# netsniff-ng/netsniff-ng

Hardware: AMD Instinct MI355X
Metric: Mpkt/s + GB/s device-resident dissect, 64B & IMIX; bit-exact fields vs ref (higher is better)
Workload: dtype u8

## Files before the change

### netsniff-ng_amd/csrc/nsd_fast.h

```cpp
#ifndef NSD_FAST_H
#define NSD_FAST_H

#include "nsd_fused.h"

namespace nsd {


constexpr int FROW = WIN1 / 4;

struct FastShared {
	alignas(16) uint32_t win[WAVES][64 * FROW];
	unsigned long long cnt[NSD_NCOUNTERS];
	uint32_t ops[32];
	uint8_t lay3[256];
	uint32_t pcnt[WAVES];
};

__device__ __forceinline__ void stage_write_sw(uint32_t *wwin, const Chunks<WIN1> &ch, int lane)
{
#pragma unroll
	for (int r = 0; r < 4; r++) {
		const int t = r * 64 + lane;
		const int q = t / 4, c = t % 4;
		const uint32_t nv = (ch.nv >> (8 * r)) & 0xFF;
		uint32_t w[4] = { ch.v[r].x, ch.v[r].y, ch.v[r].z, ch.v[r].w };
		if (nv < 16) {
#pragma unroll
			for (int j = 0; j < 4; j++) {
				const uint32_t bp = 4 * j;
				if (bp >= nv)
					w[j] = 0;
				else if (bp + 4 > nv)
					w[j] &= (1u << ((nv - bp) * 8)) - 1u;
			}
		}
		*(uint4 *)(wwin + q * FROW + ((c ^ swz_of((uint32_t)q, 4)) << 2)) = make_uint4(w[0], w[1], w[2], w[3]);
	}
}

__device__ __forceinline__ uint32_t fold_weighted(uint32_t sum, bool odd)
{
	sum = (sum >> 16) + (sum & 0xFFFF);
	sum = (sum >> 16) + (sum & 0xFFFF);
	return odd ? ((sum & 0xFF) << 8 | sum >> 8) : sum;
}

static_assert(k_plain_lay3[6] == NSD_OPS_TCP && k_plain_lay3[17] == NSD_OPS_UDP,
	      "plain_walk's protocol map differs from eth_lay3");

__device__ __forceinline__ bool plain_is(const LSrc<true, WIN1> &s, uint32_t caplen)
{
	const uint32_t r = s.m + 12, j = r >> 2, sh = r & 3;
	const uint32_t d12 = __builtin_amdgcn_alignbyte(s.dw(j + 1), s.dw(j), sh);
	const uint32_t d20 = __builtin_amdgcn_alignbyte(s.dw(j + 3), s.dw(j + 2), sh);
	const uint32_t proto = d20 >> 24;
	return caplen >= 42 && (d12 & 0xFFFFFFu) == 0x450008u && (proto == 6 || proto == 17);
}

__device__ __forceinline__ void plain_walk(const LSrc<true, WIN1> &s, uint32_t caplen, WalkOut &w)
{
	const uint32_t r = s.m + 12, j = r >> 2, sh = r & 3;
	const uint32_t w0 = s.dw(j), w1 = s.dw(j + 1), w2 = s.dw(j + 2), w3 = s.dw(j + 3), w4 = s.dw(j + 4),
		       w5 = s.dw(j + 5), w6 = s.dw(j + 6);
	const uint32_t d12 = __builtin_amdgcn_alignbyte(w1, w0, sh), d16 = __builtin_amdgcn_alignbyte(w2, w1, sh),
		       d20 = __builtin_amdgcn_alignbyte(w3, w2, sh), d24 = __builtin_amdgcn_alignbyte(w4, w3, sh),
		       d28 = __builtin_amdgcn_alignbyte(w5, w4, sh), d32 = __builtin_amdgcn_alignbyte(w6, w5, sh);
	uint32_t sum = (d12 >> 16) + (d32 & 0xFFFF);
	sum = __builtin_amdgcn_sad_u16(d16, 0u, sum);
	sum = __builtin_amdgcn_sad_u16(d20, 0u, sum);
	sum = __builtin_amdgcn_sad_u16(d24, 0u, sum);
	sum = __builtin_amdgcn_sad_u16(d28, 0u, sum);
	sum = (sum >> 16) + (sum & 0xffff);
	sum += sum >> 16;
	w.ip_csum = (uint16_t)~sum;
	const int32_t x = (int32_t)__builtin_bswap16((uint16_t)d16) - 20;
	if (x >= 0 && (uint32_t)x < caplen - 34)
		w.tail = 34 + (uint32_t)x;
	const bool tcp = (d20 >> 24) == 6;
	const int l4 = tcp ? NSD_OPS_TCP : NSD_OPS_UDP;
	w.chain = NSD_OPS_ETHERNET | NSD_OPS_IPV4 << 5 | (uint32_t)l4 << 10;
	w.offA = (uint64_t)14 << 16 | (uint64_t)34 << 32;
	w.n = 3;
	const uint32_t len = w.tail - 34, hl = tcp ? 20u : 8u;
	w.data = len >= hl ? 34 + hl : 34;
}

template <int MODE, bool CR>
__device__ __forceinline__ void fast_tiles(FastShared &sh, const uint8_t *__restrict__ frames,
					   const uint64_t *__restrict__ desc, uint32_t n, int start_id,
					   void *__restrict__ rec, const uint32_t *__restrict__ sll, uint32_t *__restrict__ side,
					   uint4 *__restrict__ list, uint32_t cap, uint32_t &ndef, uint32_t &nicmp,
					   uint32_t *__restrict__ heads, uint32_t tail0, uint32_t nheads)
{
	const int lane = threadIdx.x & 63;
	const int wv = __builtin_amdgcn_readfirstlane((int)(threadIdx.x >> 6));
	const uint32_t stride = gridDim.x * BLOCK;
	FlagCnt fc;
	auto uni = [](uint32_t x) -> uint32_t { return (uint32_t)__builtin_amdgcn_readfirstlane((int)x); };
	uint32_t base = uni(blockIdx.x * BLOCK + wv * 64);

	if (MODE != PRINT_NORM && MODE != PRINT_LESS) {
		for (; base < n; base += stride) {
			const uint32_t i = base + lane;
			fc.pkts += FlagCnt::pc(i < n);
			if (i < n) {
				const uint32_t caplen = NSD_DESC_CAPLEN(desc[i]);
				if constexpr (CR)
					__builtin_nontemporal_store(v2u{ 0u, 0u }, (v2u *)rec + i);
				else
					store_rec((uint4 *)rec, i, make_uint4(0, caplen << 16, 0, 0));
				fc.bytes += caplen;
			}
		}
		fc.flush(sh.cnt, lane);
		return;
	}
	if (base >= n)
		return;
	uint32_t *const rows = &sh.win[wv][0];
	auto dsc = [&](uint32_t b) -> uint64_t {
		return desc[b < n && b + lane < n ? b + lane : n - 1];
	};
	auto tile = [&](Chunks<WIN1> &ch, const uint64_t d0, const uint64_t dpre) {
		const uint32_t i = base + lane;
		const bool valid = i < n;
		const uint64_t off = NSD_DESC_OFF(d0);
		const uint32_t caplen = NSD_DESC_CAPLEN(d0);
		WalkOut w;
		walk_init(w, caplen, valid ? start_id : 0);
		stage_write_sw(rows, ch, lane);
		stage_load<WIN1, true>(ch, frames, dpre, lane);
		wave_sync_lds();
		uint32_t fw = FW_DONE;
		const LSrc<true, WIN1> src{ rows + lane * FROW, sh.lay3, nullptr, frames + off, caplen,
					    (uint32_t)off & 15, 0, false, swz_of((uint32_t)lane, 4) << 2 };
		const bool plain = MODE == PRINT_NORM && start_id == NSD_OPS_ETHERNET &&
				   __ballot(valid && !plain_is(src, caplen)) == 0;
		if (plain) {
			if (valid)
				plain_walk(src, caplen, w);
		} else if (valid) {
			fw = fast_walk<MODE, true>(src, caplen, w);
		}
		const bool deferred = fw != FW_DONE;
		wave_sync_lds();
		const bool done = valid && !deferred;
		if (plain) {
			const uint64_t vm = __ballot(valid), tm = __ballot(valid && w.chain >> 10 == NSD_OPS_TCP);
			const uint32_t nv = (uint32_t)__popcll(vm), nt = (uint32_t)__popcll(tm);
			if (lane == 0) {
				atomicAdd(&sh.ops[NSD_OPS_ETHERNET], nv);
				atomicAdd(&sh.ops[NSD_OPS_IPV4], nv);
				if (nt)
					atomicAdd(&sh.ops[NSD_OPS_TCP], nt);
				if (nv - nt)
					atomicAdd(&sh.ops[NSD_OPS_UDP], nv - nt);
			}
			if (valid)
				put_rec_st<CR>(rec, i, w);
			fc.pkts += nv;
			fc.ipbad += FlagCnt::pc(valid && w.ip_csum != 0);
			fc.trim += FlagCnt::pc(valid && w.tail < caplen);
			if (valid)
				fc.bytes += caplen;
			return;
		}
		if (MODE == PRINT_NORM) {
			const bool pnd = w.icmp_pend && done;
			const uint64_t pm = __ballot(pnd);
			if (pnd) {
				const uint32_t part = fold_weighted(w.icmp_sum, ((uint32_t)off + w.icmp_off) & 1);
				uint4 *e = list + (size_t)(cap - 1 - (nicmp + lanes_below(pm))) * SW;
				st_b128(e, make_uint4(i, w.icmp_off | w.icmp_len << 16, part, 0));
				st_b128(e + 1, make_uint4((uint32_t)d0, (uint32_t)(d0 >> 32), 0, 0));
			}
			nicmp = uni(nicmp + (uint32_t)__popcll(pm));
		}
		{
			uint32_t key = done ? w.chain : 0xFFFFFFFFu;
			for (int it = 0;; it++) {
				const uint64_t pm = __ballot(key != 0xFFFFFFFFu);
				if (!pm)
					break;
				if (it == 2) {
					if (key != 0xFFFFFFFFu)
						for (uint32_t k = 0; k < w.n; k++)
							atomicAdd(&sh.ops[(key >> (5 * k)) & 31], 1u);
					break;
				}
				const int leader = __ffsll((unsigned long long)pm) - 1;
				const uint32_t lk = __shfl(key, leader, 64);
				const uint64_t m = __ballot(key == lk);
				if (lane == leader) {
					const uint32_t cnt = (uint32_t)__popcll(m);
					for (uint32_t k = 0, nl = w.n; k < nl; k++)
						atomicAdd(&sh.ops[(lk >> (5 * k)) & 31], cnt);
				}
				if (key == lk)
					key = 0xFFFFFFFFu;
			}
		}
		if (CR && side && done && (w.flags & NSD_F_HOST)) {
			st_b32(side + i, w.data);
			w.flags |= NSD_F_LEAF_END;
		}
		if (done)
			put_rec_st<CR>(rec, i, w);
		fc.add(w, caplen, done);
		const uint64_t dm = __ballot(deferred);
		if (dm) {
			if (deferred) {
				if (fw == FW_RESTART) {
					walk_init(w, caplen, start_id);
					if (start_id == NSD_OPS_SLL) {
						const uint32_t w0 = sll ? sll[5 * (size_t)i] : 0u;
						const uint32_t w2 = sll ? sll[5 * (size_t)i + 2] : 0u;
						const uint32_t proto = __builtin_bswap16((uint16_t)(w0 >> 16));
						w.chain = NSD_OPS_SLL;
						w.n = 1;
						atomicAdd(&sh.ops[NSD_OPS_SLL], 1u);
						w.id = sll_next(w2 & 0xFFFF, proto, MODE, c_lay2h.e[NSD_L2H(proto)]);
					}
				} else {
					for (uint32_t k = 0; k < w.n; k++)
						atomicAdd(&sh.ops[(w.chain >> (5 * k)) & 31], 1u);
				}
				uint4 *e = list + (size_t)(ndef + lanes_below(dm)) * SW;
				st_b128(e, make_uint4(i, w.data | w.tail << 16,
						      (uint32_t)w.ip_csum | (uint32_t)w.flags << 16 | w.n << 24 |
							      (uint32_t)w.id << 27,
						      w.chain));
				const uint32_t offs = CR ? 0u
							 : ((uint32_t)(w.offA >> 16) & 0xFF) | ((uint32_t)(w.offA >> 32) & 0xFF) << 8 |
								   ((uint32_t)(w.offA >> 48) & 0xFF) << 16 | (w.offB & 0xFF) << 24;
				st_b128(e + 1, make_uint4((uint32_t)d0, (uint32_t)(d0 >> 32), offs, 0));
			}
			ndef = uni(ndef + (uint32_t)__popcll(dm));
		}
	};
	const uint32_t ntiles = (n + 63) / 64;
	const uint32_t slim = heads ? tail0 * 64 : n;
	uint32_t cur = heads ? blockIdx.x % nheads : 0, tries = nheads > 1 ? 0 : NSD_TAIL_TRIES;
	bool more = heads != nullptr, asked = false;
	uint32_t gv = 0;
	auto draw = [&]() {
		if (lane == 0) {
			uint32_t z;
			asm volatile("v_mov_b32 %0, 0" : "=v"(z));
			gv = atomicAdd(heads + LINE_WORDS * cur + z, 1u);
		}
	};
	auto ask = [&]() {
		asked = more && ndef + nicmp + 64u * 7 <= cap;
		more = asked;
		if (asked)
			draw();
	};
	uint32_t second = n;
	auto take = [&]() -> uint32_t {
		if (!asked)
			return n;
		asked = false;
		auto tile_of = [&]() -> uint32_t {
			const uint32_t k = (uint32_t)__builtin_amdgcn_readfirstlane((int)gv);
			return tail0 + 2 * (cur + k * nheads);
		};
		uint32_t t = tile_of();
		auto next = [&]() {
			tries++;
			cur = cur + 1 == nheads ? 0 : cur + 1;
			draw();
			t = tile_of();
		};
		static_assert(NSD_TAIL_TRIES == 3, "take(): one nested test per try");
		if (t >= ntiles && tries < NSD_TAIL_TRIES) {
			next();
			if (t >= ntiles && tries < NSD_TAIL_TRIES) {
				next();
				if (t >= ntiles && tries < NSD_TAIL_TRIES)
					next();
			}
		}
		if (t >= ntiles) {
			more = false;
			return n;
		}
		second = t + 1 < ntiles ? (t + 1) * 64 : n;
		if (second == n)
			more = false;
		return t * 64;
	};
	uint32_t nxt = uni(base + 3 * stride);
	auto step = [&]() -> uint32_t {
		uint32_t b;
		if (nxt < slim) {
			b = nxt;
			nxt = uni(nxt + stride);
			if (nxt >= slim)
				ask();
		} else if (second < n) {
			b = second;
			second = n;
		} else {
			b = take();
			ask();
		}
		return b;
	};
	uint32_t b1 = base + stride < slim ? base + stride : n, b2 = base + 2 * stride < slim ? base + 2 * stride : n;
	uint64_t d0 = dsc(base), d1 = dsc(b1), d2 = dsc(b2);
	Chunks<WIN1> chA, chB;
	stage_load<WIN1, true>(chA, frames, d0, lane);
	stage_load<WIN1, true>(chB, frames, d1, lane);
	for (;;) {
		uint32_t b3 = uni(step());
		uint64_t d3 = dsc(b3);
		tile(chA, d0, d2);
		d0 = d1;
		d1 = d2;
		d2 = d3;
		base = uni(b1);
		b1 = b2;
		b2 = b3;
		if (base >= n)
			break;
		b3 = uni(step());
		d3 = dsc(b3);
		tile(chB, d0, d2);
		d0 = d1;
		d1 = d2;
		d2 = d3;
		base = uni(b1);
		b1 = b2;
		b2 = b3;
		if (base >= n)
			break;
	}
	drain_stores();
	if (lane == 0 && ndef + nicmp > cap)
		atomicAdd(&sh.cnt[NSD_CNT_LISTOVF], 1ull);
	fc.flush(sh.cnt, lane);
}

template <int U, bool CR>
__device__ __forceinline__ void fast_icmp_pass(FastShared &sh, const uint8_t *__restrict__ frames,
					       const uint64_t *__restrict__ desc, void *__restrict__ rec,
					       const uint4 *__restrict__ lists, uint32_t cap)
{
	const int lane = threadIdx.x & 63;
	const int wv = threadIdx.x >> 6;
	const uint32_t sub = lane & 3, grp = lane >> 2;
	uint32_t bad = 0;
	for (int l = 0; l < WAVES; l++) {
		const uint32_t cnt = sh.pcnt[l];
		const uint4 *list = lists + ((size_t)blockIdx.x * WAVES + l) * cap * SW;
		for (uint32_t k0 = 64 * ((wv + l) % WAVES); k0 < cnt; k0 += 64 * WAVES) {
			const bool on = k0 + lane < cnt;
			const uint4 *ep = list + (size_t)(cap - 1 - (k0 + lane)) * SW;
			const uint4 e = on ? ep[0] : make_uint4(0, 0, 0, 0);
			const uint32_t i = e.x;
			const uint64_t a = (on ? NSD_DESC_OFF((uint64_t)ep[1].y << 32 | ep[1].x) : 0) + (e.y & 0xFFFF);
			const uint32_t nb = e.y >> 16;
			for (uint32_t q = 0; q < 64 && k0 + q < cnt; q += 16) {
				const int src = (int)(q + grp);
				const uint32_t alo = __shfl((uint32_t)a, src, 64);
				const uint32_t ahi = __shfl((uint32_t)(a >> 32), src, 64);
				const uint32_t mnb = __shfl(nb, src, 64);
				const uint32_t part = __shfl(e.z, src, 64);
				const bool mon = k0 + (uint32_t)src < cnt;
				const uint32_t s0 = alo & 15, endb = s0 + mnb;
				const uint32_t nch = mon ? (endb + 15) >> 4 : 0u;
				const uint4 *base = (const uint4 *)(frames + ((((uint64_t)ahi << 32) | alo) & ~15ull));
				uint32_t sum = sub == 0 ? part : 0u;
				const uint32_t je = sub == 0 ? 0u : nch - 1;
				if ((sub == 0 && nch > 0) || (sub == 1 && nch > 1))
					sum += csum_chunk(base[je], 16 * je, s0, endb);
				for (uint32_t j = 1 + sub; __ballot(j + 1 < nch); j += 4 * U) {
					uint4 v[U];
#pragma unroll
					for (int u = 0; u < U; u++) {
						const uint32_t jj = j + 4 * u;
						v[u] = jj + 1 < nch ? base[jj] : make_uint4(0, 0, 0, 0);
					}
#pragma unroll
					for (int u = 0; u < U; u++) {
						sum = sum_halves(v[u].x, sum);
						sum = sum_halves(v[u].y, sum);
						sum = sum_halves(v[u].z, sum);
						sum = sum_halves(v[u].w, sum);
					}
				}
				sum = (sum >> 16) + (sum & 0xffff);
				sum += __shfl_xor(sum, 1, 64);
				sum += __shfl_xor(sum, 2, 64);
				const uint32_t mi = __shfl(i, src, 64);
				const bool isbad = mon && sub == 0 && csum_final(sum) != 0;
				if (isbad) {
					uint8_t *nf = (uint8_t *)rec + nflags_at<CR>(mi);
					*nf = *nf | NSD_F_ICMP_BAD;
				}
				bad += FlagCnt::pc(isbad);
			}
		}
	}
	if (lane == 0 && bad)
		atomicAdd(&sh.cnt[NSD_CNT_ICMP_BAD], (unsigned long long)bad);
}

template <int MODE, bool CR>
__device__ __forceinline__ void walk_lists(Shared &sh, uint32_t *s_touch, const uint8_t *__restrict__ frames,
					   const uint64_t *__restrict__ desc, uint32_t n, void *__restrict__ rec,
					   uint32_t *__restrict__ ext, uint32_t ext_words, uint32_t *__restrict__ ext_used,
					   uint32_t chunk, unsigned long long *__restrict__ counters,
					   const uint4 *__restrict__ list, uint32_t cnt, uint64_t *__restrict__ pend,
					   uint32_t region)
{
	if (threadIdx.x < 64)
		sh.step[threadIdx.x] = threadIdx.x < 32 ? c_step[threadIdx.x] : c_lay2h.e[threadIdx.x - 32];
	if (threadIdx.x < 32)
		sh.ops[threadIdx.x] = 0;
	if (threadIdx.x < 2 * WAVES)
		sh.wc[threadIdx.x >> 1][threadIdx.x & 1] = 0;
	block_init(sh.cnt, sh.lay3);
	const int lane = threadIdx.x & 63, wv = threadIdx.x >> 6;
	const uint32_t gw = blockIdx.x * WAVES + wv;
	Pending pq{ pend + (size_t)gw * (region / WAVES), region / WAVES, 0, 0 };
	const bool side = CR && ext_words >= n;
	const GenSink<CR> g{ ext, ext_words, ext_used, chunk, &sh.wc[wv][0], sh.ops, &sh.lay[wv][0],
			     CR ? n : 0u, side ? ext : nullptr };
	FlagCnt fc;
	Walker wk;
	walk_init(wk.w, 0, 0);
	wk.d = 0;
	wk.i = 0;
	wk.wb = 0;
	wk.wl = 0;
	wk.have = false;
	wk.stage = false;
	WalkOut pw;
	walk_init(pw, 0, 0);
	RingSt rs;
	rs.init();

	auto load = [&](uint32_t k0, uint4 &x0, uint4 &x1) {
		x0 = x1 = make_uint4(0, 0, 0, 0);
		if (k0 + lane < cnt) {
			const uint4 *e = list + (size_t)(k0 + lane) * SW;
			x0 = e[0];
			x1 = e[1];
		}
	};
	uint4 c0, c1, n0, n1;
	load(0, c0, c1);
	load(64, n0, n1);
	for (uint32_t k0 = 0; k0 < cnt; k0 += 64) {
		{
			const uint64_t d = (uint64_t)n1.y << 32 | n1.x;
			const uint32_t m = (uint32_t)NSD_DESC_OFF(d) & 15, caplen = NSD_DESC_CAPLEN(d);
			const uint32_t wb = ((n0.y & 0xFFFF) + m) & ~15u;
			const bool on = k0 + 64 + lane < cnt && wb < caplen + m;
			const uint64_t a = (uint64_t)frames + (NSD_DESC_OFF(d) & ~15ull) + wb;
			const bool two = on && (a & 127) != 0 && wb + (128 - (uint32_t)(a & 127)) < caplen + m;
			if (on)
				__builtin_amdgcn_global_load_lds((const void *)(a & ~127ull),
								 (__attribute__((address_space(3))) void *)s_touch, 4, 0, 0);
			if (two)
				__builtin_amdgcn_global_load_lds((const void *)((a & ~127ull) + 128),
								 (__attribute__((address_space(3))) void *)s_touch, 4, 0, 0);
		}
		uint4 m0, m1;
		load(k0 + 128, m0, m1);
		bool pnd = k0 + lane < cnt;
		const uint32_t pi = c0.x;
		const uint64_t pd = (uint64_t)c1.y << 32 | c1.x;
		walk_init(pw, c0.y >> 16, (int)(c0.z >> 27));
		pw.data = c0.y & 0xFFFF;
		pw.ip_csum = (uint16_t)c0.z;
		pw.flags = (uint8_t)(c0.z >> 16);
		pw.n = (c0.z >> 24) & 7;
		pw.chain = c0.w;
		if (!CR) {
			pw.offA = (uint64_t)(c1.z & 0xFF) << 16 | (uint64_t)((c1.z >> 8) & 0xFF) << 32 |
				  (uint64_t)((c1.z >> 16) & 0xFF) << 48;
			pw.offB = c1.z >> 24;
		}
		walkers<MODE, CR, false>(sh, rs, frames, rec, g, pq, fc, wk, pnd, pw, pi, pd, false);
		c0 = n0;
		c1 = n1;
		n0 = m0;
		n1 = m1;
	}
	{
		bool none = false;
		if (__ballot(wk.have))
			walkers<MODE, CR, false>(sh, rs, frames, rec, g, pq, fc, wk, none, pw, 0, 0, true);
	}
	fc.flush(sh.cnt, lane);
	leaf_pass<MODE, CR>(frames, desc, rec, ext, pq);
	if (lane == 0)
		sh.pcnt[wv] = pq.npend;
	if (MODE == PRINT_NORM) {
		__syncthreads();
		icmp_pass<NSD_CSUM_U, CR>(sh, frames, desc, rec, pend, region);
	}
	block_flush(sh.cnt, counters);
	if (threadIdx.x < 32 && sh.ops[threadIdx.x])
		atomicAdd(&counters[NSD_CNT_OPS + threadIdx.x], (unsigned long long)sh.ops[threadIdx.x]);
}

template <int MODE, bool CR>
__global__ __launch_bounds__(BLOCK, CR ? NSD_FAST_MINW : NSD_FAST_MINW_FULL) void dissect_fast(
	const uint8_t *__restrict__ frames, const uint64_t *__restrict__ desc, uint32_t n, int start_id,
	void *__restrict__ rec, unsigned long long *__restrict__ counters, uint4 *__restrict__ lists, uint32_t cap,
	const uint32_t *__restrict__ sll, uint32_t *__restrict__ side, unsigned long long *__restrict__ sched,
	uint32_t *__restrict__ ext, uint32_t ext_words, uint32_t *__restrict__ ext_used, uint32_t chunk,
	uint64_t *__restrict__ pend, uint32_t region, uint32_t *__restrict__ heads, uint32_t tail0, uint32_t nheads)
{
	union FastLds {
		FastShared f;
		Shared w;
	};
	__shared__ FastLds su;
	FastShared &sh = su.f;
	if (threadIdx.x < 32)
		sh.ops[threadIdx.x] = 0;
	block_init(sh.cnt, sh.lay3);
	const int lane = threadIdx.x & 63, wv = threadIdx.x >> 6;
	const uint32_t gw = blockIdx.x * WAVES + wv;
	uint4 *const list = lists + (size_t)gw * cap * SW;
	uint32_t ndef = 0, nicmp = 0;
	fast_tiles<MODE, CR>(sh, frames, desc, n, start_id, rec, sll, side, list, cap, ndef, nicmp, heads, tail0, nheads);
	if (lane == 0) {
		sh.pcnt[wv] = nicmp;
		if (sched && ndef)
			atomicAdd(&sched[0], (unsigned long long)ndef);
		if (sched && nicmp)
			atomicAdd(&sched[1], (unsigned long long)nicmp);
	}
	if (MODE == PRINT_NORM) {
		__syncthreads();
		fast_icmp_pass<NSD_FAST_CSUM_U, CR>(sh, frames, desc, rec, lists, cap);
	}
	block_flush(sh.cnt, counters);
	if (threadIdx.x < 32 && sh.ops[threadIdx.x])
		atomicAdd(&counters[NSD_CNT_OPS + threadIdx.x], (unsigned long long)sh.ops[threadIdx.x]);
	if constexpr (MODE == PRINT_NORM || MODE == PRINT_LESS) {
		const bool tail = __syncthreads_or(ndef != 0);
		if (heads && threadIdx.x == 0 && atomicAdd(heads + LINE_WORDS * nheads, 1u) == gridDim.x - 1) {
			for (uint32_t h = 0; h <= nheads; h++)
				atomicExch(heads + LINE_WORDS * h, 0u);
		}
		if (tail) {
			__shared__ uint32_t s_touch[64];
			walk_lists<MODE, CR>(su.w, s_touch, frames, desc, n, rec, ext, ext_words, ext_used, chunk, counters,
					     list, min(ndef, cap), pend, region);
		}
	}
}

}

#endif
```

### netsniff-ng_amd/csrc/nsd_internal.h

```cpp
#ifndef NSD_INTERNAL_H
#define NSD_INTERNAL_H

#include <hip/hip_runtime_api.h>
#include <stddef.h>
#include <stdint.h>
#include <stdio.h>

#include <string>
#include <vector>

#include "../../include/netsniff_dissect.h"

#define NSD_HIDDEN __attribute__((visibility("hidden")))

NSD_HIDDEN inline bool hip_ok(hipError_t e, const char *what)
{
	if (e != hipSuccess) {
		fprintf(stderr, "netsniff-dissect: %s: %s\n", what, hipGetErrorString(e));
		return false;
	}
	return true;
}

template <class T>
NSD_HIDDEN inline bool grow(T *&p, size_t &cap, size_t need)
{
	if (need <= cap)
		return true;
	if (p)
		(void)hipFree(p);
	p = nullptr;
	cap = 0;
	const size_t want = need + need / 4 + 64;
	if (!hip_ok(hipMalloc(&p, want * sizeof(T)), "hipMalloc"))
		return false;
	cap = want;
	return true;
}

inline size_t batch_extent(const nsd_desc_t *desc, size_t n)
{
	size_t used = 0;
	for (size_t j = 0; j < n; j++) {
		const size_t e = NSD_DESC_OFF(desc[j]) + NSD_DESC_CAPLEN(desc[j]);
		used = e > used ? e : used;
	}
	return used;
}

extern "C" int nsd_launch_dissect_rec(const uint8_t *d_frames, const uint64_t *d_desc, const void *d_sll,
				      uint32_t n, int start_id, int mode, void *d_rec, int compact, uint32_t *d_ext,
				      uint32_t ext_words, uint32_t *d_ext_used, uint64_t *d_counters, void *d_ws,
				      int grid, hipStream_t stream);
extern "C" size_t nsd_launch_workspace_bytes(uint32_t n);
extern "C" int nsd_launch_workspace_layout(uint32_t n, uint32_t blocks, int compact, uint64_t *out);
extern "C" int nsd_last_tail_shared(void);

NSD_HIDDEN int nsd_start_for(int linktype);
extern "C" NSD_HIDDEN int nsd_pipe_retarget(nsd_pipe *p, int linktype, int mode);

extern "C" NSD_HIDDEN long nsd_flow_feed_host(nsd_flow_table *t, const uint8_t *frames, size_t frames_len,
					      const nsd_desc_t *desc, const nsd_sll_t *sll, uint32_t n, int linktype,
					      int mode, const nsd_bpf_prog *filter, const uint64_t *ts, uint64_t *ts_max,
					      uint64_t base);
extern "C" NSD_HIDDEN int nsd_flow_feed_records(nsd_flow_table *t, const uint8_t *frames, size_t frames_len,
						const nsd_desc_t *desc, uint32_t n, const nsd_rec *rec,
						const uint32_t *ext, uint32_t ext_words, const uint64_t *ts, uint64_t base);
NSD_HIDDEN long nsd_flow_expire_rows(nsd_flow_table *t, uint64_t before, uint32_t flags, uint32_t max,
				     std::vector<nsd_flow> &rows, uint64_t *stats);
NSD_HIDDEN long nsd_flow_expire_rows_ts(nsd_flow_table *t, uint64_t before_ns, uint32_t flags, uint32_t max,
					std::vector<nsd_flowt> &rows, uint64_t *stats);

extern "C" NSD_HIDDEN void nsd_if_cache_reset(void);
extern "C" NSD_HIDDEN void nsd_replay_release(void);
extern "C" NSD_HIDDEN void nsd_device_ctx_release(void);

namespace nsd {
bool render_layer(std::string &s, const uint8_t *pkt, uint32_t caplen, int id, uint32_t start, uint32_t tail,
		  int mode, uint16_t ip_csum, bool icmp_bad, const nsd_sll_t *sll, uint32_t &data,
		  uint32_t &ntail, bool &next);
void render_hex(std::string &s, const uint8_t *pkt, uint32_t caplen, uint32_t from, uint32_t len);
void render_ascii(std::string &s, const uint8_t *pkt, uint32_t caplen, uint32_t from, uint32_t len);
void format_frame_hdr(std::string &s, const nsd_frame_hdr_t &fh, const nsd_sll_t *sll, const uint8_t *pkt,
		      uint32_t caplen, int linktype, int mode, uint64_t count);
int render_packet_cpu(std::string &text, const uint8_t *packet, size_t len, int linktype, int mode,
		      const nsd_sll_t *sll);
int format_replay_part(std::string &s, const uint8_t *frames, const nsd_desc_t *desc, const nsd_frame_hdr_t *fh,
		       const nsd_sll_t *sll, const nsd_crec *rec, const uint32_t *ext, uint64_t count0, uint32_t lo,
		       uint32_t hi, int linktype, int mode);
int cpu_step(int mode, const uint8_t *pkt, uint32_t caplen, int id, uint32_t &data, uint32_t &tail,
	     uint16_t &ip_csum, uint8_t &flags, const nsd_sll_t *sll);
void cpu_count_packet(const uint8_t *pkt, uint32_t caplen, int linktype, int mode, const nsd_sll_t *sll,
		      uint64_t *counters);
}

#endif
```

### netsniff-ng_amd/csrc/nsd_launch.h

```cpp
#ifndef NSD_LAUNCH_H
#define NSD_LAUNCH_H

#include <hip/hip_runtime.h>
#include <stddef.h>
#include <stdint.h>

#include "nsd_internal.h"

#ifndef NSD_WIN2
#define NSD_WIN2 128
#endif
#ifndef NSD_CSUM_U
#define NSD_CSUM_U 12
#endif
#ifndef NSD_FAST_CSUM_U
#define NSD_FAST_CSUM_U 8
#endif
#ifndef NSD_CSUM_LANES
#define NSD_CSUM_LANES 8
#endif
#ifndef NSD_MINW
#define NSD_MINW 4
#endif
#ifndef NSD_FAST_MINW
#define NSD_FAST_MINW 4
#endif
#ifndef NSD_FAST_MINW_FULL
#define NSD_FAST_MINW_FULL 4
#endif
#ifndef NSD_FAST_BPC
#define NSD_FAST_BPC 3
#endif
#ifndef NSD_FAST_BPC_SMALL
#define NSD_FAST_BPC_SMALL 2
#endif
#ifndef NSD_GROUP_BLOCKS
#define NSD_GROUP_BLOCKS 4u
#endif
#ifndef NSD_L2PF
#define NSD_L2PF 16
#endif
#ifndef NSD_REFILL
#define NSD_REFILL 16
#endif
#ifndef NSD_WIN_AHEAD
#define NSD_WIN_AHEAD 32
#endif
#ifndef NSD_SCHED_SAMPLE
#define NSD_SCHED_SAMPLE 32
#endif
#ifndef NSD_TAIL_DIV
#define NSD_TAIL_DIV 2
#endif
#ifndef NSD_TAIL_MIN_ROUNDS
#define NSD_TAIL_MIN_ROUNDS 16
#endif
#ifndef NSD_TAIL_HEAD_BLOCKS
#define NSD_TAIL_HEAD_BLOCKS 16
#endif
#ifndef NSD_TAIL_TRIES
#define NSD_TAIL_TRIES 3u
#endif
#ifndef NSD_SMALL_FRAME
#define NSD_SMALL_FRAME 128
#endif

constexpr uint32_t NSD_MAX_GRID = 4096;
constexpr uint32_t NSD_TAIL_HEADS_MAX = 256;

namespace nsd {

constexpr int BLOCK = 256;
constexpr int WAVES = BLOCK / 64;

constexpr int SW = 2;
constexpr int LIST_SLOT_BYTES = SW * 16;
constexpr int PEND_BYTES = 8;
constexpr int LINE_BYTES = 128;
constexpr int LINE_WORDS = LINE_BYTES / 4;
constexpr uint32_t fused_region(uint32_t region, bool compact)
{
	return compact ? 2 * region + WAVES * 4 * 64 : region;
}
constexpr int PAIR_BYTES = 16;
constexpr uint32_t TAIL_CAP_DIV = 5;

typedef void (*kfn)(const uint8_t *, const uint64_t *, uint32_t, int, void *, uint32_t *, uint32_t, uint32_t *,
		    uint32_t, unsigned long long *, uint64_t *, uint32_t, const uint32_t *, unsigned long long *,
		    uint32_t *, uint32_t);
typedef void (*ffn)(const uint8_t *, const uint64_t *, uint32_t, int, void *, unsigned long long *, uint4 *,
		    uint32_t, const uint32_t *, uint32_t *, unsigned long long *, uint32_t *, uint32_t, uint32_t *,
		    uint32_t, uint64_t *, uint32_t, uint32_t *, uint32_t, uint32_t);
NSD_HIDDEN kfn fused_kernel(bool compact, int mi, bool ring);
NSD_HIDDEN ffn fast_kernel(bool compact, int mi);
NSD_HIDDEN void (*zero_tiles_kernel())(uint32_t *, uint32_t);

struct WsLayout {
	uint32_t blocks;
	uint32_t rounds;
	struct Carve {
		uint32_t cap;
		size_t lists_bytes, pend_at, pend_bytes;
	};
	Carve st, sh;
	bool sh_fits;
	uint32_t fused_region;
	size_t gtiles_at, pair_at, total;
	uint32_t tail_rounds, tail_heads;
};
NSD_HIDDEN WsLayout ws_layout(uint32_t n, uint32_t blocks, bool compact);

}

#endif
```

### netsniff-ng_amd/csrc/nsd_launch.hip

```cpp
#include <hip/hip_runtime.h>
#include <stdint.h>

#include <atomic>
#include <mutex>

#include "nsd_internal.h"
#include "nsd_launch.h"

namespace {
constexpr int MAX_DEV = 16;
struct Sched {
	bool init = false, fused = false, pending = false, small = false;
	bool walky = false;
	bool sampled_once = false;
	bool recorded = false;
	bool discard = false;
	int launches = 0;
	int last = 0;
	bool last_shared = false;
	uint64_t sampled = 0;
	unsigned long long *host = nullptr;
	hipEvent_t ev = nullptr;
	int cus = 0;
};
Sched g_sched[MAX_DEV];
std::mutex g_sched_mu;
int g_sched_force = 0;
int g_ring_force = 0;
std::atomic<int> g_grid_cap{ 0 };
std::atomic<int> g_debug_fill{ -1 };

int cur_dev()
{
	int d = 0;
	if (hipGetDevice(&d) != hipSuccess || d < 0 || d >= MAX_DEV)
		d = 0;
	return d;
}

struct Plan {
	bool fused, sample, small, prio, ring;
	int cus;
};
Plan sched_plan(uint32_t n, unsigned long long *pair, const uint64_t *counters, hipStream_t stream, bool capturing)
{
	std::lock_guard<std::mutex> g(g_sched_mu);
	const int dev = cur_dev();
	Sched &S = g_sched[dev];
	if (!S.cus) {
		int cus = 0;
		if (hipDeviceGetAttribute(&cus, hipDeviceAttributeMultiprocessorCount, dev) != hipSuccess || cus < 1)
			cus = 256;
		S.cus = cus;
	}
	Plan p{ false, false, false, true, true, S.cus };
	const bool landed = !capturing && S.pending && S.recorded && hipEventQuery(S.ev) == hipSuccess;
	if (landed && S.discard) {
		S.pending = S.recorded = S.discard = false;
	} else if (landed) {
		const double rd = S.sampled ? (double)S.host[0] / (double)S.sampled : 0.0;
		const double ri = S.sampled ? (double)S.host[1] / (double)S.sampled : 0.0;
		S.fused = S.fused ? rd > 0.05 || ri > 0.05 : rd > 0.15 || ri > 0.10;
		const uint64_t pk = S.host[4] - S.host[2], by = S.host[5] - S.host[3];
		if (pk)
			S.small = by <= (uint64_t)NSD_SMALL_FRAME * pk;
		S.walky = rd > 0.25;
		S.sampled_once = true;
		S.pending = false;
		S.recorded = false;
	}
	if (!S.init && !capturing) {
		S.init = true;
		if (hipHostMalloc((void **)&S.host, 64, hipHostMallocDefault) != hipSuccess ||
		    hipEventCreateWithFlags(&S.ev, hipEventDisableTiming) != hipSuccess)
			S.host = nullptr;
	}
	p.fused = g_sched_force ? g_sched_force == NSD_SCHED_FUSED : S.fused;
	p.small = S.small;
	p.prio = !S.walky;
	p.ring = g_ring_force ? g_ring_force == 1 : !S.sampled_once || S.walky;
	if (!capturing && ++S.launches >= NSD_SCHED_SAMPLE && !S.pending && S.host && pair && counters &&
	    hipMemsetAsync(pair, 0, nsd::PAIR_BYTES, stream) == hipSuccess &&
	    hipMemcpyAsync(S.host + 2, counters + NSD_CNT_PKTS, 16, hipMemcpyDeviceToHost, stream) == hipSuccess) {
		p.sample = true;
		S.launches = 0;
		S.sampled = n;
		S.pending = true;
		S.recorded = false;
	}
	return p;
}

void sched_ran(bool fused, bool shared)
{
	std::lock_guard<std::mutex> g(g_sched_mu);
	Sched &S = g_sched[cur_dev()];
	S.last = fused ? NSD_SCHED_FUSED : NSD_SCHED_SPLIT;
	S.last_shared = shared;
}

constexpr int NSD_TAIL_SETS = 64;
struct TailSet {
	int dev;
	hipStream_t stream;
	uint32_t *heads;
};
TailSet g_tail[NSD_TAIL_SETS];
int g_ntail = 0;

uint32_t *tail_set(hipStream_t stream)
{
	if (stream == hipStreamPerThread)
		return nullptr;
	std::lock_guard<std::mutex> g(g_sched_mu);
	const int dev = cur_dev();
	for (int k = 0; k < g_ntail; k++)
		if (g_tail[k].dev == dev && g_tail[k].stream == stream)
			return g_tail[k].heads;
	if (g_ntail == NSD_TAIL_SETS)
		return nullptr;
	const size_t bytes = (size_t)(NSD_TAIL_HEADS_MAX + 1) * nsd::LINE_BYTES;
	uint32_t *h = nullptr;
	if (hipMalloc((void **)&h, bytes) != hipSuccess) {
		(void)hipGetLastError();
		return nullptr;
	}
	if (hipMemsetAsync(h, 0, bytes, stream) != hipSuccess) {
		(void)hipGetLastError();
		(void)hipFree(h);
		return nullptr;
	}
	g_tail[g_ntail++] = TailSet{ dev, stream, h };
	return h;
}

void sched_fail(Sched &S, hipStream_t stream)
{
	S.discard = true;
	if (hipEventRecord(S.ev, stream) == hipSuccess) {
		S.recorded = true;
		return;
	}
	(void)hipStreamSynchronize(stream);
	S.pending = S.recorded = S.discard = false;
}

void sched_sampled(unsigned long long *pair, const uint64_t *counters, hipStream_t stream)
{
	std::lock_guard<std::mutex> g(g_sched_mu);
	Sched &S = g_sched[cur_dev()];
	if (hipMemcpyAsync(S.host, pair, nsd::PAIR_BYTES, hipMemcpyDeviceToHost, stream) != hipSuccess ||
	    hipMemcpyAsync(S.host + 4, counters + NSD_CNT_PKTS, 16, hipMemcpyDeviceToHost, stream) != hipSuccess ||
	    hipEventRecord(S.ev, stream) != hipSuccess) {
		sched_fail(S, stream);
		return;
	}
	S.recorded = true;
}

void sched_abort(hipStream_t stream)
{
	std::lock_guard<std::mutex> g(g_sched_mu);
	sched_fail(g_sched[cur_dev()], stream);
}
}

extern "C" int nsd_set_schedule(int sched)
{
	if (sched != NSD_SCHED_ADAPTIVE && sched != NSD_SCHED_SPLIT && sched != NSD_SCHED_FUSED)
		return NSD_ERR_ARG;
	std::lock_guard<std::mutex> g(g_sched_mu);
	const int prev = g_sched_force;
	g_sched_force = sched;
	return prev;
}

extern "C" int nsd_set_record_ring(int mode)
{
	if (mode < 0 || mode > 2)
		return NSD_ERR_ARG;
	std::lock_guard<std::mutex> g(g_sched_mu);
	const int prev = g_ring_force;
	g_ring_force = mode;
	return prev;
}

extern "C" int nsd_set_grid_cap(int blocks)
{
	if (blocks < 0)
		return NSD_ERR_ARG;
	return g_grid_cap.exchange(blocks);
}

extern "C" int nsd_set_debug_fill(int byte)
{
	if (byte < -1 || byte > 255)
		return NSD_ERR_ARG;
	return g_debug_fill.exchange(byte);
}

extern "C" int nsd_last_tail_shared(void)
{
	std::lock_guard<std::mutex> g(g_sched_mu);
	return g_sched[cur_dev()].last_shared ? 1 : 0;
}

extern "C" int nsd_last_schedule(void)
{
	std::lock_guard<std::mutex> g(g_sched_mu);
	return g_sched[cur_dev()].last;
}

static size_t align256(size_t x) { return (x + 255) & ~(size_t)255; }

static_assert(NSD_TAIL_DIV == 0 || (NSD_TAIL_DIV >= 2 && NSD_TAIL_MIN_ROUNDS >= 16 && NSD_TAIL_HEAD_BLOCKS >= 16),
	      "fast_tiles: a static front of more than three rounds, and its liveness argument");

nsd::WsLayout nsd::ws_layout(uint32_t n, uint32_t blocks, bool compact)
{
	WsLayout L;
	const uint32_t want = ((n + 63) / 64 + WAVES - 1) / WAVES;
	if (blocks > NSD_MAX_GRID)
		blocks = NSD_MAX_GRID;
	L.blocks = blocks < want ? blocks : want;
	const uint64_t stride = (uint64_t)L.blocks * BLOCK;
	L.rounds = (uint32_t)((n + stride - 1) / stride);
	const size_t slots = ((size_t)n + (size_t)NSD_MAX_GRID * BLOCK + 1) & ~(size_t)1;
	L.gtiles_at = align256(align256(LIST_SLOT_BYTES * slots) + align256((size_t)NSD_MAX_GRID * WAVES * PEND_BYTES) +
			       2 * PEND_BYTES * slots);
	L.pair_at = L.gtiles_at + (size_t)NSD_MAX_GRID * LINE_BYTES;
	L.total = L.pair_at + 256;
	const size_t nlists = (size_t)L.blocks * WAVES;
	auto carve = [&](uint32_t cap) {
		const size_t lists_bytes = LIST_SLOT_BYTES * nlists * cap;
		return WsLayout::Carve{ cap, lists_bytes, align256(lists_bytes) + align256(nlists * PEND_BYTES),
					PEND_BYTES * nlists * cap };
	};
	L.st = carve(L.rounds * 64);
	L.sh = carve(L.st.cap + L.st.cap / TAIL_CAP_DIV);
	L.sh_fits = L.sh.pend_at + L.sh.pend_bytes <= L.gtiles_at;
	L.fused_region = fused_region(L.rounds * BLOCK, compact);
	L.tail_rounds = 0;
	if (NSD_TAIL_DIV != 0 && L.sh_fits && L.rounds >= NSD_TAIL_MIN_ROUNDS) {
		uint32_t t = L.rounds / NSD_TAIL_DIV;
		if (!t)
			t = 1;
		L.tail_rounds = t + ((L.rounds - t) & 1);
	}
	uint32_t h = L.blocks / NSD_TAIL_HEAD_BLOCKS;
	if (h >= 8)
		h &= ~7u;
	if (h > NSD_TAIL_HEADS_MAX)
		h = NSD_TAIL_HEADS_MAX & ~7u;
	L.tail_heads = h ? h : 1;
	return L;
}

extern "C" size_t nsd_launch_workspace_bytes(uint32_t n)
{
	return nsd::ws_layout(n, 1, false).total;
}

extern "C" int nsd_launch_workspace_layout(uint32_t n, uint32_t blocks, int compact, uint64_t *out)
{
	if (!n || !blocks || !out)
		return NSD_ERR_ARG;
	const nsd::WsLayout L = nsd::ws_layout(n, blocks, compact != 0);
	const uint64_t v[20] = { L.total, 0, (uint64_t)nsd::PEND_BYTES * L.fused_region * L.blocks,
				 L.gtiles_at, compact ? (uint64_t)nsd::LINE_BYTES * L.blocks : 0,
				 L.pair_at, (uint64_t)nsd::PAIR_BYTES,
				 0, L.st.lists_bytes, L.st.pend_at, L.st.pend_bytes,
				 0, L.sh.lists_bytes, L.sh.pend_at, L.sh.pend_bytes,
				 L.sh_fits, L.st.cap, L.sh.cap, L.tail_rounds, L.tail_heads };
	for (int k = 0; k < 20; k++)
		out[k] = v[k];
	return 0;
}

extern "C" int nsd_launch_dissect_rec(const uint8_t *d_frames, const uint64_t *d_desc, const void *d_sll,
				      uint32_t n, int start_id, int mode, void *d_rec, int compact, uint32_t *d_ext,
				      uint32_t ext_words, uint32_t *d_ext_used, uint64_t *d_counters, void *d_ws,
				      int grid, hipStream_t stream)
{
	using namespace nsd;
	if (n == 0)
		return 0;
	const int mi = mode == PRINT_NORM ? 0 : mode == PRINT_LESS ? 1 : 2;
	const int ci = compact ? 1 : 0;
	if (ext_words > NSD_EXT_POOL_MAX_WORDS)
		ext_words = NSD_EXT_POOL_MAX_WORDS;
	auto chunk_for = [&](uint32_t blocks) {
		const uint64_t per = (uint64_t)ext_words / (2ull * blocks * WAVES);
		const uint32_t lo = NSD_EXT_WORDS(NSD_EXT_MAX_LAYERS), hi = 512 * NSD_EXT_WORDS(16);
		return (uint32_t)(per < lo ? lo : per > hi ? hi : per) & ~3u;
	};
	auto occupancy = [&](const void *f, std::atomic<int> &slot, int dflt) {
		int occ = slot.load(std::memory_order_relaxed);
		if (!occ) {
			if (hipOccupancyMaxActiveBlocksPerMultiprocessor(&occ, f, BLOCK, 0) != hipSuccess || occ < 1)
				occ = dflt;
			slot.store(occ, std::memory_order_relaxed);
		}
		return occ;
	};
	if (grid <= 0)
		grid = g_grid_cap.load(std::memory_order_relaxed);
	hipStreamCaptureStatus cs = hipStreamCaptureStatusNone;
	const bool cs_known = hipStreamIsCapturing(stream, &cs) == hipSuccess;
	const bool capturing = cs_known && cs != hipStreamCaptureStatusNone;
	const WsLayout L0 = ws_layout(n, 1, compact != 0);
	const int fill = g_debug_fill.load(std::memory_order_relaxed);
	if (fill >= 0 && cs_known && !capturing) {
		if (hipMemsetAsync(d_rec, fill, (size_t)n * (compact ? sizeof(nsd_crec) : sizeof(nsd_rec)), stream) != hipSuccess ||
		    (d_ext && ext_words && hipMemsetAsync(d_ext, fill, (size_t)ext_words * 4, stream) != hipSuccess) ||
		    (d_ws && hipMemsetAsync(d_ws, fill, L0.total, stream) != hipSuccess))
			return -2;
	}
	uint8_t *const ws = (uint8_t *)d_ws;
	unsigned long long *const pair = ws ? (unsigned long long *)(ws + L0.pair_at) : nullptr;
	const Plan plan = sched_plan(n, mi != 2 ? pair : nullptr, d_counters, stream, capturing);
	const int s_cus = plan.cus;
	unsigned long long *const sched = plan.sample ? pair : nullptr;
	auto launched = [&]() {
		if (hipGetLastError() == hipSuccess)
			return true;
		if (sched)
			sched_abort(stream);
		return false;
	};
	uint32_t *heads = nullptr;
	if (mi != 2 && plan.fused) {
		static std::atomic<int> s_occ[2][3], s_rocc[2];
		const bool ring = plan.ring && ci == 1 && mi < 2;
		const kfn f = fused_kernel(ci, mi, ring);
		std::atomic<int> &occ_slot = ring ? s_rocc[mi] : s_occ[ci][mi];
		const WsLayout L = ws_layout(n, grid > 0 ? (uint32_t)grid : (uint32_t)(s_cus * occupancy((const void *)f, occ_slot, 4)),
					     compact != 0);
		uint32_t *const gtiles = (uint32_t *)(ws + L.gtiles_at);
		if (compact) {
			hipLaunchKernelGGL(zero_tiles_kernel(), dim3((L.blocks + 255) / 256), dim3(256), 0, stream, gtiles,
					   L.blocks);
			if (!launched())
				return -2;
		}
		hipLaunchKernelGGL(f, dim3(L.blocks), dim3(BLOCK), 0, stream, d_frames, d_desc, n, start_id, d_rec, d_ext,
				   ext_words, d_ext_used, chunk_for(L.blocks), (unsigned long long *)d_counters,
				   (uint64_t *)ws, L.fused_region, (const uint32_t *)d_sll, sched, gtiles,
				   plan.prio ? 1u : 0u);
	} else {
		static std::atomic<int> s_focc[2][3];
		const ffn f = fast_kernel(ci, mi);
		uint32_t fcap = grid > 0 ? (uint32_t)grid : (uint32_t)(s_cus * occupancy((const void *)f, s_focc[ci][mi], 8));
		const int bpc = plan.small ? NSD_FAST_BPC_SMALL : NSD_FAST_BPC;
		if (grid <= 0 && bpc > 0 && fcap > (uint32_t)(s_cus * bpc))
			fcap = (uint32_t)(s_cus * bpc);
		const WsLayout L = ws_layout(n, fcap, compact != 0);
		const uint32_t trounds = mi != 2 && !capturing ? L.tail_rounds : 0;
		heads = trounds ? tail_set(stream) : nullptr;
		const WsLayout::Carve &cv = heads ? L.sh : L.st;
		const uint32_t tail0 = heads ? (L.rounds - trounds) * L.blocks * WAVES : 0;
		uint32_t *side = compact && d_ext && ext_words >= n ? d_ext : nullptr;
		hipLaunchKernelGGL(f, dim3(L.blocks), dim3(BLOCK), 0, stream, d_frames, d_desc, n, start_id, d_rec,
				   (unsigned long long *)d_counters, (uint4 *)ws, cv.cap, (const uint32_t *)d_sll, side, sched,
				   d_ext, ext_words, d_ext_used, chunk_for(L.blocks), (uint64_t *)(ws + cv.pend_at),
				   cv.cap * WAVES, heads, tail0, L.tail_heads);
	}
	if (!launched())
		return -2;
	sched_ran(plan.fused, heads != nullptr);
	if (sched)
		sched_sampled(sched, d_counters, stream);
	return 0;
}
```

Measured before the change: 88110.

## Add pair/single tail ticket scheme and skip idle ICMP pass

Tail work-stealing tickets can now hand out single tiles after a precomputed number of tile pairs, so the end of the grid is balanced at finer granularity. The number of single slots comes from a host-side knob that defaults to zero, which keeps pair-only behaviour by default. The kernel epilogue is also reordered: the tail barrier and head reset move earlier, the ICMP pass is skipped when no wave queued ICMP work, and the counter flush is inlined. This removes a barrier and pass for blocks without ICMP, at the cost of extra synchronisation when a tail walk is needed.

```diff
diff --git a/netsniff-ng_amd/csrc/nsd_fast.h b/netsniff-ng_amd/csrc/nsd_fast.h
--- a/netsniff-ng_amd/csrc/nsd_fast.h
+++ b/netsniff-ng_amd/csrc/nsd_fast.h
@@ -85,12 +85,23 @@
 	w.data = len >= hl ? 34 + hl : 34;
 }
 
+template <int K, class Again, class Next>
+__device__ __forceinline__ void nested_tries(const Again &again, const Next &next)
+{
+	if constexpr (K > 0) {
+		if (again()) {
+			next();
+			nested_tries<K - 1>(again, next);
+		}
+	}
+}
+
 template <int MODE, bool CR>
 __device__ __forceinline__ void fast_tiles(FastShared &sh, const uint8_t *__restrict__ frames,
 					   const uint64_t *__restrict__ desc, uint32_t n, int start_id,
 					   void *__restrict__ rec, const uint32_t *__restrict__ sll, uint32_t *__restrict__ side,
 					   uint4 *__restrict__ list, uint32_t cap, uint32_t &ndef, uint32_t &nicmp,
-					   uint32_t *__restrict__ heads, uint32_t tail0, uint32_t nheads)
+					   uint32_t *__restrict__ heads, uint32_t tail0, uint32_t nheads, uint32_t pairs)
 {
 	const int lane = threadIdx.x & 63;
 	const int wv = __builtin_amdgcn_readfirstlane((int)(threadIdx.x >> 6));
@@ -261,9 +272,12 @@
 		if (!asked)
 			return n;
 		asked = false;
+		bool pair = false;
 		auto tile_of = [&]() -> uint32_t {
 			const uint32_t k = (uint32_t)__builtin_amdgcn_readfirstlane((int)gv);
-			return tail0 + 2 * (cur + k * nheads);
+			const TailTicket tk = tail_ticket(k, cur, tail0, nheads, pairs);
+			pair = tk.pair;
+			return tk.tile;
 		};
 		uint32_t t = tile_of();
 		auto next = [&]() {
@@ -272,22 +286,12 @@
 			draw();
 			t = tile_of();
 		};
-		static_assert(NSD_TAIL_TRIES == 3, "take(): one nested test per try");
-		if (t >= ntiles && tries < NSD_TAIL_TRIES) {
-			next();
-			if (t >= ntiles && tries < NSD_TAIL_TRIES) {
-				next();
-				if (t >= ntiles && tries < NSD_TAIL_TRIES)
-					next();
-			}
-		}
+		nested_tries<(int)NSD_TAIL_TRIES>([&]() { return t >= ntiles && tries < NSD_TAIL_TRIES; }, next);
 		if (t >= ntiles) {
 			more = false;
 			return n;
 		}
-		second = t + 1 < ntiles ? (t + 1) * 64 : n;
-		if (second == n)
-			more = false;
+		second = pair ? (t + 1) * 64 : n;
 		return t * 64;
 	};
 	uint32_t nxt = uni(base + 3 * stride);
@@ -514,7 +518,8 @@
 	void *__restrict__ rec, unsigned long long *__restrict__ counters, uint4 *__restrict__ lists, uint32_t cap,
 	const uint32_t *__restrict__ sll, uint32_t *__restrict__ side, unsigned long long *__restrict__ sched,
 	uint32_t *__restrict__ ext, uint32_t ext_words, uint32_t *__restrict__ ext_used, uint32_t chunk,
-	uint64_t *__restrict__ pend, uint32_t region, uint32_t *__restrict__ heads, uint32_t tail0, uint32_t nheads)
+	uint64_t *__restrict__ pend, uint32_t region, uint32_t *__restrict__ heads, uint32_t tail0, uint32_t nheads,
+	uint32_t pairs)
 {
 	union FastLds {
 		FastShared f;
@@ -529,7 +534,8 @@
 	const uint32_t gw = blockIdx.x * WAVES + wv;
 	uint4 *const list = lists + (size_t)gw * cap * SW;
 	uint32_t ndef = 0, nicmp = 0;
-	fast_tiles<MODE, CR>(sh, frames, desc, n, start_id, rec, sll, side, list, cap, ndef, nicmp, heads, tail0, nheads);
+	fast_tiles<MODE, CR>(sh, frames, desc, n, start_id, rec, sll, side, list, cap, ndef, nicmp, heads, tail0, nheads,
+			     pairs);
 	if (lane == 0) {
 		sh.pcnt[wv] = nicmp;
 		if (sched && ndef)
@@ -537,20 +543,23 @@
 		if (sched && nicmp)
 			atomicAdd(&sched[1], (unsigned long long)nicmp);
 	}
-	if (MODE == PRINT_NORM) {
+	const bool tail = __syncthreads_or(ndef != 0);
+	if (heads && threadIdx.x == 0 && atomicAdd(heads + LINE_WORDS * nheads, 1u) == gridDim.x - 1) {
+		for (uint32_t h = 0; h <= nheads; h++)
+			atomicExch(heads + LINE_WORDS * h, 0u);
+	}
+	if (MODE == PRINT_NORM && (sh.pcnt[0] | sh.pcnt[1] | sh.pcnt[2] | sh.pcnt[3]) != 0) {
+		fast_icmp_pass<NSD_FAST_CSUM_U, CR>(sh, frames, desc, rec, lists, cap);
 		__syncthreads();
-		fast_icmp_pass<NSD_FAST_CSUM_U, CR>(sh, frames, desc, rec, lists, cap);
-	}
-	block_flush(sh.cnt, counters);
+	}
+	for (int k = threadIdx.x; k < NSD_NCOUNTERS; k += BLOCK)
+		if (sh.cnt[k])
+			atomicAdd(&counters[k], sh.cnt[k]);
 	if (threadIdx.x < 32 && sh.ops[threadIdx.x])
 		atomicAdd(&counters[NSD_CNT_OPS + threadIdx.x], (unsigned long long)sh.ops[threadIdx.x]);
 	if constexpr (MODE == PRINT_NORM || MODE == PRINT_LESS) {
-		const bool tail = __syncthreads_or(ndef != 0);
-		if (heads && threadIdx.x == 0 && atomicAdd(heads + LINE_WORDS * nheads, 1u) == gridDim.x - 1) {
-			for (uint32_t h = 0; h <= nheads; h++)
-				atomicExch(heads + LINE_WORDS * h, 0u);
-		}
 		if (tail) {
+			__syncthreads();
 			__shared__ uint32_t s_touch[64];
 			walk_lists<MODE, CR>(su.w, s_touch, frames, desc, n, rec, ext, ext_words, ext_used, chunk, counters,
 					     list, min(ndef, cap), pend, region);
diff --git a/netsniff-ng_amd/csrc/nsd_internal.h b/netsniff-ng_amd/csrc/nsd_internal.h
--- a/netsniff-ng_amd/csrc/nsd_internal.h
+++ b/netsniff-ng_amd/csrc/nsd_internal.h
@@ -54,6 +54,11 @@
 				      int grid, hipStream_t stream);
 extern "C" size_t nsd_launch_workspace_bytes(uint32_t n);
 extern "C" int nsd_launch_workspace_layout(uint32_t n, uint32_t blocks, int compact, uint64_t *out);
+extern "C" int nsd_launch_tail_layout(uint32_t n, uint32_t blocks, int compact, uint64_t *out);
+extern "C" int nsd_set_tail_singles(int x2);
+extern "C" uint32_t nsd_launch_tail_pairs(uint32_t tiles, uint32_t nheads, uint32_t singles);
+extern "C" uint32_t nsd_launch_tail_ticket(uint32_t k, uint32_t head, uint32_t tail0, uint32_t nheads, uint32_t pairs,
+					   int *pair);
 extern "C" int nsd_last_tail_shared(void);
 
 NSD_HIDDEN int nsd_start_for(int linktype);
diff --git a/netsniff-ng_amd/csrc/nsd_launch.h b/netsniff-ng_amd/csrc/nsd_launch.h
--- a/netsniff-ng_amd/csrc/nsd_launch.h
+++ b/netsniff-ng_amd/csrc/nsd_launch.h
@@ -58,6 +58,9 @@
 #ifndef NSD_TAIL_HEAD_BLOCKS
 #define NSD_TAIL_HEAD_BLOCKS 16
 #endif
+#ifndef NSD_TAIL_SINGLES_X2
+#define NSD_TAIL_SINGLES_X2 0
+#endif
 #ifndef NSD_TAIL_TRIES
 #define NSD_TAIL_TRIES 3u
 #endif
@@ -85,12 +88,29 @@
 constexpr int PAIR_BYTES = 16;
 constexpr uint32_t TAIL_CAP_DIV = 5;
 
+struct TailTicket {
+	uint32_t tile;
+	bool pair;
+};
+__host__ __device__ inline TailTicket tail_ticket(uint32_t k, uint32_t head, uint32_t tail0, uint32_t nheads,
+						  uint32_t pairs)
+{
+	if (k < pairs)
+		return TailTicket{ tail0 + 2 * (head + k * nheads), true };
+	return TailTicket{ tail0 + 2 * pairs * nheads + head + (k - pairs) * nheads, false };
+}
+constexpr uint32_t tail_pairs(uint32_t tiles, uint32_t nheads, uint32_t singles)
+{
+	return (uint64_t)singles * nheads >= tiles ? 0
+						   : (uint32_t)((tiles - (uint64_t)singles * nheads) / (2ull * nheads));
+}
+
 typedef void (*kfn)(const uint8_t *, const uint64_t *, uint32_t, int, void *, uint32_t *, uint32_t, uint32_t *,
 		    uint32_t, unsigned long long *, uint64_t *, uint32_t, const uint32_t *, unsigned long long *,
 		    uint32_t *, uint32_t);
 typedef void (*ffn)(const uint8_t *, const uint64_t *, uint32_t, int, void *, unsigned long long *, uint4 *,
 		    uint32_t, const uint32_t *, uint32_t *, unsigned long long *, uint32_t *, uint32_t, uint32_t *,
-		    uint32_t, uint64_t *, uint32_t, uint32_t *, uint32_t, uint32_t);
+		    uint32_t, uint64_t *, uint32_t, uint32_t *, uint32_t, uint32_t, uint32_t);
 NSD_HIDDEN kfn fused_kernel(bool compact, int mi, bool ring);
 NSD_HIDDEN ffn fast_kernel(bool compact, int mi);
 NSD_HIDDEN void (*zero_tiles_kernel())(uint32_t *, uint32_t);
@@ -107,6 +127,7 @@
 	uint32_t fused_region;
 	size_t gtiles_at, pair_at, total;
 	uint32_t tail_rounds, tail_heads;
+	uint32_t tail0, ntiles, tail_pairs, tail_singles;
 };
 NSD_HIDDEN WsLayout ws_layout(uint32_t n, uint32_t blocks, bool compact);
 
diff --git a/netsniff-ng_amd/csrc/nsd_launch.hip b/netsniff-ng_amd/csrc/nsd_launch.hip
--- a/netsniff-ng_amd/csrc/nsd_launch.hip
+++ b/netsniff-ng_amd/csrc/nsd_launch.hip
@@ -28,6 +28,7 @@
 int g_sched_force = 0;
 int g_ring_force = 0;
 std::atomic<int> g_grid_cap{ 0 };
+std::atomic<int> g_tail_singles{ NSD_TAIL_SINGLES_X2 };
 std::atomic<int> g_debug_fill{ -1 };
 
 int cur_dev()
@@ -190,6 +191,13 @@
 	if (blocks < 0)
 		return NSD_ERR_ARG;
 	return g_grid_cap.exchange(blocks);
+}
+
+extern "C" int nsd_set_tail_singles(int x2)
+{
+	if (x2 < 0 || x2 > 16)
+		return NSD_ERR_ARG;
+	return g_tail_singles.exchange(x2);
 }
 
 extern "C" int nsd_set_debug_fill(int byte)
@@ -253,6 +261,10 @@
 	if (h > NSD_TAIL_HEADS_MAX)
 		h = NSD_TAIL_HEADS_MAX & ~7u;
 	L.tail_heads = h ? h : 1;
+	L.ntiles = (n + 63) / 64;
+	L.tail0 = (L.rounds - L.tail_rounds) * L.blocks * WAVES;
+	L.tail_singles = L.blocks / L.tail_heads * WAVES * (uint32_t)g_tail_singles.load(std::memory_order_relaxed) / 2;
+	L.tail_pairs = L.tail_rounds ? tail_pairs(L.ntiles - L.tail0, L.tail_heads, L.tail_singles) : 0;
 	return L;
 }
 
@@ -275,6 +287,31 @@
 	for (int k = 0; k < 20; k++)
 		out[k] = v[k];
 	return 0;
+}
+
+extern "C" int nsd_launch_tail_layout(uint32_t n, uint32_t blocks, int compact, uint64_t *out)
+{
+	if (!n || !blocks || !out)
+		return NSD_ERR_ARG;
+	const nsd::WsLayout L = nsd::ws_layout(n, blocks, compact != 0);
+	const uint64_t v[6] = { L.tail0, L.ntiles, L.tail_heads, L.tail_pairs, L.tail_singles, L.tail_rounds };
+	for (int k = 0; k < 6; k++)
+		out[k] = v[k];
+	return 0;
+}
+
+extern "C" uint32_t nsd_launch_tail_pairs(uint32_t tiles, uint32_t nheads, uint32_t singles)
+{
+	return nheads ? nsd::tail_pairs(tiles, nheads, singles) : 0;
+}
+
+extern "C" uint32_t nsd_launch_tail_ticket(uint32_t k, uint32_t head, uint32_t tail0, uint32_t nheads, uint32_t pairs,
+					   int *pair)
+{
+	const nsd::TailTicket t = nsd::tail_ticket(k, head, tail0, nheads, pairs);
+	if (pair)
+		*pair = t.pair ? 1 : 0;
+	return t.tile;
 }
 
 extern "C" int nsd_launch_dissect_rec(const uint8_t *d_frames, const uint64_t *d_desc, const void *d_sll,
@@ -358,12 +395,12 @@
 		const uint32_t trounds = mi != 2 && !capturing ? L.tail_rounds : 0;
 		heads = trounds ? tail_set(stream) : nullptr;
 		const WsLayout::Carve &cv = heads ? L.sh : L.st;
-		const uint32_t tail0 = heads ? (L.rounds - trounds) * L.blocks * WAVES : 0;
+		const uint32_t tail0 = heads ? L.tail0 : 0;
 		uint32_t *side = compact && d_ext && ext_words >= n ? d_ext : nullptr;
 		hipLaunchKernelGGL(f, dim3(L.blocks), dim3(BLOCK), 0, stream, d_frames, d_desc, n, start_id, d_rec,
 				   (unsigned long long *)d_counters, (uint4 *)ws, cv.cap, (const uint32_t *)d_sll, side, sched,
 				   d_ext, ext_words, d_ext_used, chunk_for(L.blocks), (uint64_t *)(ws + cv.pend_at),
-				   cv.cap * WAVES, heads, tail0, L.tail_heads);
+				   cv.cap * WAVES, heads, tail0, L.tail_heads, L.tail_pairs);
 	}
 	if (!launched())
 		return -2;
```

After: 88580, median of 6. No clear change (+0.5%).
